# google-research/se3ds

Hardware: AMD Instinct MI355X
Metric: panoramas/sec (G+D train step) at 512x1024 RGB-D (higher is better)
Workload: dtype bf16; 1 GPU; configs/highres 512x1024 full GAN step train_g_d (G+D+hinge+depth+wc losses, clip, Adam, EMA), ResNet-101 gen_dims 128, per-GPU batch 8, d_step_per_g_step 1; per_gpu_batch=8, global_batch=8, parallelism=dp1

## Files before the change

### include/se3ds_hip.h

```cpp
#ifndef SE3DS_HIP_H_
#define SE3DS_HIP_H_

#include <stddef.h>
#include <stdint.h>

#ifdef __cplusplus
extern "C" {
#endif

#define SE3DS_OK 0
#define SE3DS_E_BADSHAPE (-1)
#define SE3DS_E_BADDTYPE (-2)
#define SE3DS_E_WORKSPACE (-3)
#define SE3DS_E_LAUNCH (-4)
#define SE3DS_E_UNSUPPORTED (-5)

#define SE3DS_F32 0
#define SE3DS_I32 1
#define SE3DS_U8 2
#define SE3DS_BF16 3
#define SE3DS_FEAT_BYTE_RANGE 0x100
#define SE3DS_XYZ1_ONES_PRESET 0x200

const char* se3ds_version(void);
// ... 237 lines not shown
                         void* stream);
int se3ds_upsample2x_fwd(const void* x, int dtype, int n, int h, int w, int c, void* y,
                         void* stream);
int se3ds_upsample2x_bwd(const void* dy, int dtype, int n, int h, int w, int c, void* dx,
                         void* stream);
int se3ds_copy_channels(const void* src, int src_dtype, int src_c, int src_c0, void* dst,
                        int dst_dtype, int dst_c, int dst_c0, int ncopy, int64_t rows,
                        void* stream);
int se3ds_fill(void* p, int dtype, int64_t n, float value, void* stream);
int se3ds_quantize(const void* in, int in_dtype, int64_t n, int pre_clamp, float pre_lo,
                   float pre_hi, float mul, float div, float lo, float hi, void* out, int out_dtype,
                   void* stream);
int se3ds_pad2d(const void* x, int dtype, int n, int h, int w, int c, int pad, int mode, int wrap_w,
                float value, void* y, void* stream);
int se3ds_head_fwd(const void* x, int dtype, int64_t n, int kind, float* y, void* stream);
int se3ds_head_bwd(const float* dy, const float* y, const void* x, int dtype, int64_t n, int kind,
                   void* dx, void* stream);

int se3ds_sample_sum(const float* a, const float* b, const float* m, int n, int64_t p, int c,
                     int mode, float* out, float* workspace , void* stream);
int se3ds_l1_grad(const float* a, const float* b, const float* m, const float* m2,
                  const float* coef, int n, int64_t p, int c, int mode, float* grad, void* stream);
int se3ds_recip_clamp(const float* sums, int n, float scale, float* out, void* stream);
int se3ds_hinge(const void* logits, int dtype, int64_t half, float cd, float cg, float* sums,
                void* dlog_d, void* dlog_g, void* stream);

int se3ds_multi_sqnorm(const float* grads, const int64_t* chunks, int64_t nchunks,
                       const int64_t* tensor_chunk_start, int ntensors, float* partial,
                       float* sqnorm, void* stream);
int se3ds_multi_clip_by_norm(float* grads, const int64_t* chunks, int64_t nchunks,
                             const float* sqnorm, int ntensors, float clip_norm,
                             float* mean_norm_out, void* stream);
int se3ds_mean_clipped_norm(const float* sqnorm, int ntensors, float clip_norm, float* out,
                            void* stream);
int se3ds_multi_adam_keras(float* params, const float* grads, float* m, float* v, int64_t n,
                           float lr, float beta1, float beta2, float eps, int64_t step,
                           void* stream);
int se3ds_multi_adam_keras_ema(float* params, const float* grads, float* m, float* v, int64_t n,
                               float lr, float beta1, float beta2, float eps, int64_t step,
                               float* ema, float one_minus_decay, void* stream);
int se3ds_multi_clip_adam_keras_ema(float* params, const float* grads, float* m, float* v,
                                    const int64_t* chunks, int64_t nchunks, const float* sqnorm,
                                    float clip_norm, const int64_t* tensor_sn, float lr, float beta1,
                                    float beta2, float eps, int64_t step, float* ema,
                                    float one_minus_decay, void* stream);
int se3ds_multi_ema(float* ema, const float* vars, int64_t n, float one_minus_decay, void* stream);

int se3ds_spectral_table_fields(void);
int se3ds_spectral_part_rows(void);
int se3ds_spectral_vpart_len(void);
int se3ds_spectral_power_iter(const int64_t* table, int nlayers, int training, void* stream);
int se3ds_spectral_bwd_fixup(const int64_t* table, int nlayers, void* stream);
int se3ds_spectral_bwd_dots(const int64_t* table, int nlayers, void* stream);
int se3ds_multi_sqnorm_sn(const float* grads, const int64_t* chunks, int64_t nchunks,
                          const int64_t* tensor_chunk_start, int ntensors, float* partial,
                          float* sqnorm, const int64_t* tensor_sn, int tensor_base, void* stream);
int se3ds_multi_clip_by_norm_sn(float* grads, const int64_t* chunks, int64_t nchunks,
                                const float* sqnorm, int ntensors, float clip_norm,
                                float* mean_norm_out, const int64_t* tensor_sn, void* stream);


int se3ds_input_transform(const uint8_t* image, const uint8_t* proj_image, const uint16_t* depth,
                          const uint16_t* proj_depth, const uint8_t* proj_mask,
                          const uint8_t* blurred_mask, const uint8_t* segmentation,
                          const int32_t* iparams, const float* fparams, int n, int h0, int w0, int h,
                          int w, float* o_image, float* o_proj_image, float* o_proj_mask,
                          float* o_proj_depth, float* o_depth, float* o_blurred, int32_t* o_seg,
                          void* stream);

int se3ds_video_transform(const float* image, const uint8_t* segmentation,
                          const uint8_t* pd_segmentation, const float* depth, const float* pd_depth,
                          const int32_t* hmode, const float* hband, int n, int t, int h0, int w0,
                          int h, int w, float* o_original, float* o_image, uint8_t* o_seg,
                          uint8_t* o_pd_seg, float* o_depth, float* o_pd_depth, void* stream);

int se3ds_re10k_extent(const uint8_t* visible_mask, int n, int h0, int w0, int32_t* extents,
                       void* stream);
int se3ds_re10k_extent_vector_bytes(const uint8_t* visible_mask, int w0);

int se3ds_re10k_transform(const uint8_t* image, const uint8_t* proj_image, const uint16_t* depth,
                          const uint16_t* proj_depth, const uint8_t* proj_mask,
                          const uint8_t* visible_mask, const uint8_t* segmentation,
                          const int32_t* extents, const int32_t* iparams, const float* fparams,
                          int n, int h0, int w0, int h, int w, float* o_image, float* o_proj_image,
                          float* o_proj_mask, float* o_proj_depth, float* o_depth, float* o_blurred,
                          int32_t* o_seg, int32_t* o_bbox, int32_t* o_status, void* stream);

int se3ds_png_unfilter(const uint8_t* src, int64_t src_bytes, const int64_t* table,
                       const int64_t* host_table, int n, void* stream);
int se3ds_png_unfilter_fields(void);
int se3ds_png_unfilter_max_row_bytes(void);

int se3ds_png_inflate(const uint8_t* buf, int64_t buf_bytes, uint8_t* workspace,
                      int64_t workspace_bytes, const int64_t* host_table, int n,
                      int32_t* status_dev, void* stream);
int se3ds_png_inflate_fields(void);
int se3ds_png_inflate_ring_bytes(void);

int se3ds_jpeg_decode(const uint8_t* buf, int64_t buf_bytes, uint8_t* workspace,
                      int64_t workspace_bytes, const int64_t* host_images, int n_images,
                      const int64_t* host_segments, int n_segments, int32_t* status_dev, int phases,
                      void* stream);
size_t se3ds_jpeg_decode_workspace_bytes(const int64_t* host_images, int n_images);
int se3ds_jpeg_decode_fields(void);
int se3ds_jpeg_decode_segment_fields(void);
int se3ds_jpeg_decode_lanes(void);
// ... 167 lines not shown
```

### se3ds_amd/csrc/optim.hip

```cpp
#include "common.h"
#include <cmath>

namespace se3ds {
namespace {

constexpr int kB = 256;

__global__ void __launch_bounds__(kB)
chunk_sqsum_kernel(const float* __restrict__ g, const int64_t* __restrict__ chunks,
                   float* __restrict__ partial, const int64_t* __restrict__ tensor_sn) {
  __shared__ float sh[kB / 64];
  const int64_t start = chunks[blockIdx.x * 3 + 1], len = chunks[blockIdx.x * 3 + 2];
  if (tensor_sn && tensor_sn[chunks[blockIdx.x * 3]] != 0) {
    if (threadIdx.x == 0) partial[blockIdx.x] = 0.f;
    return;
  }
  float s = 0.f;
  const float* gp = g + start;
  const int64_t n4 = (((uintptr_t)gp & 15) == 0) ? (len >> 2) : 0;
  float s1 = 0.f, s2 = 0.f, s3 = 0.f;
  for (int64_t i = threadIdx.x; i < n4; i += kB) {
    const float4 v = reinterpret_cast<const float4*>(gp)[i];
    s += v.x * v.x;
    s1 += v.y * v.y;
// ... 310 lines not shown
  }
  dot = wave_sum(dot);
  __syncthreads();
  if ((threadIdx.x & 63) == 0) sh[threadIdx.x >> 6] = dot;
  __syncthreads();
  if (threadIdx.x == 0) {
    float sigma = (sh[0] + sh[1]) + (sh[2] + sh[3]);
    sig[0] = sigma;
    sig[1] = 1.0f / (sigma + SN_EPS);
  }
  float vn = 0.f;
  for (int i = 0; i < SN_RB; ++i) vn += vpart[i];
  const float inv_vn = 1.0f / (sqrtf(vn) + SN_EPS);
  for (int64_t k = threadIdx.x; k < K; k += kB) v[k] = v[k] * inv_vn;
}

__global__ void __launch_bounds__(kB)
sn_dot_kernel(const int64_t* __restrict__ tab) {
  const int64_t* L = tab + (int64_t)blockIdx.y * SN_F;
  const float* W = (const float*)L[0];
  float* vpart = (float*)L[6];
  const float* G = (const float*)L[9];
  const int64_t n = L[7] * L[8];
  __shared__ float sh[kB / 64];
  float s = 0.f;
  for (int64_t i = (int64_t)blockIdx.x * kB + threadIdx.x; i < n; i += (int64_t)SN_RB * kB)
    s += G[i] * W[i];
  s = wave_sum(s);
  if ((threadIdx.x & 63) == 0) sh[threadIdx.x >> 6] = s;
  __syncthreads();
  if (threadIdx.x == 0) vpart[blockIdx.x] = (sh[0] + sh[1]) + (sh[2] + sh[3]);
}

__global__ void __launch_bounds__(kB)
sn_fix_kernel(const int64_t* __restrict__ tab) {
  const int64_t* L = tab + (int64_t)blockIdx.y * SN_F;
  const float* v = (const float*)L[2];
  const float* uhat = (const float*)L[3];
  const float* sig = (const float*)L[4];
  const float* vpart = (const float*)L[6];
  float* G = (float*)L[9];
  const int C = (int)L[8];
  const int64_t n = L[7] * C;
  const float dot = sn_dot_gw(vpart);
  const float inv = sig[1];
  const float coef = inv * inv * dot;
  for (int64_t i = (int64_t)blockIdx.x * kB + threadIdx.x; i < n; i += (int64_t)SN_RB * kB) {
    int64_t k = i / C;
    int c = (int)(i - k * C);
    G[i] = inv * G[i] - coef * v[k] * uhat[c];
  }
}

__global__ void __launch_bounds__(kB)
sn_dots_kernel(const int64_t* __restrict__ tab) {
  const int64_t* L = tab + (int64_t)blockIdx.y * SN_F;
  const float* W = (const float*)L[0];
  const float* v = (const float*)L[2];
  const float* uhat = (const float*)L[3];
  float* vpart = (float*)L[6];
  const float* G = (const float*)L[9];
  const int64_t K = L[7];
  const int C = (int)L[8];
  __shared__ float sh[3][kB / 64];
  const int lane = threadIdx.x & 63, wave = threadIdx.x >> 6;
  float dot = 0.f, gg = 0.f, gvu = 0.f;
  const bool vec = (C & 3) == 0 && ((((uintptr_t)G | (uintptr_t)W | (uintptr_t)uhat) & 15) == 0);
  for (int64_t k = (int64_t)blockIdx.x * 4 + wave; k < K; k += (int64_t)SN_RB * 4) {
    const float vk = v[k];
    float row = 0.f;
    if (vec) {
      const float4* G4 = reinterpret_cast<const float4*>(G + k * C);
      const float4* W4 = reinterpret_cast<const float4*>(W + k * C);
      const float4* U4 = reinterpret_cast<const float4*>(uhat);
      for (int c = lane; c < (C >> 2); c += 64) {
        const float4 gv = G4[c], wv = W4[c], uv = U4[c];
        dot += (gv.x * wv.x + gv.y * wv.y) + (gv.z * wv.z + gv.w * wv.w);
        gg += (gv.x * gv.x + gv.y * gv.y) + (gv.z * gv.z + gv.w * gv.w);
        row += (gv.x * uv.x + gv.y * uv.y) + (gv.z * uv.z + gv.w * uv.w);
      }
    } else {
      for (int c = lane; c < C; c += 64) {
        const float gv = G[k * C + c];
        dot += gv * W[k * C + c];
        gg += gv * gv;
        row += gv * uhat[c];
      }
    }
    gvu += row * vk;
  }
  dot = wave_sum(dot);
  gg = wave_sum(gg);
  gvu = wave_sum(gvu);
  if (lane == 0) { sh[0][wave] = dot; sh[1][wave] = gg; sh[2][wave] = gvu; }
  __syncthreads();
  if (threadIdx.x < 3) {
    const float* q = sh[threadIdx.x];
    vpart[threadIdx.x * SN_RB + blockIdx.x] = (q[0] + q[1]) + (q[2] + q[3]);
  }
  if (blockIdx.x == 0) {
    __syncthreads();
    float nv = 0.f, nu = 0.f;
    for (int64_t k = threadIdx.x; k < K; k += kB) nv += v[k] * v[k];
    for (int c = threadIdx.x; c < C; c += kB) nu += uhat[c] * uhat[c];
    nv = wave_sum(nv);
    nu = wave_sum(nu);
    if (lane == 0) { sh[0][wave] = nv; sh[1][wave] = nu; }
    __syncthreads();
    if (threadIdx.x < 2) {
      const float* q = sh[threadIdx.x];
      vpart[3 * SN_RB + threadIdx.x] = (q[0] + q[1]) + (q[2] + q[3]);
    }
  }
}

__global__ void __launch_bounds__(kB)
sn_sqnorm_kernel(const int64_t* __restrict__ tensor_sn, int tensor_base, int T,
                 float* __restrict__ sqnorm) {
  for (int t = blockIdx.x * kB + threadIdx.x; t < T; t += gridDim.x * kB) {
    const int64_t* L = (const int64_t*)tensor_sn[tensor_base + t];
    if (L == nullptr) continue;
    const float* sig = (const float*)L[4];
    const float* vpart = (const float*)L[6];
    const float dot = sn_dot_gw(vpart);
    double gg = 0.0, gvu = 0.0;
    for (int i = 0; i < SN_RB; ++i) {
      gg += (double)vpart[SN_RB + i];
      gvu += (double)vpart[2 * SN_RB + i];
    }
// ... 88 lines not shown
  float alpha = adam_alpha(lr, beta1, beta2, step);
  hipLaunchKernelGGL(adam_ema_kernel, dim3(grid_for(n, kB)), dim3(kB), 0, as_stream(stream), params,
                     grads, m, v, n, alpha, beta1, beta2, eps, ema, one_minus_decay);
  return check_launch("multi_adam_keras_ema");
}

int se3ds_multi_clip_adam_keras_ema(float* params, const float* grads, float* m, float* v,
                                    const int64_t* chunks, int64_t nchunks, const float* sqnorm,
                                    float clip_norm, const int64_t* tensor_sn, float lr, float beta1,
                                    float beta2, float eps, int64_t step, float* ema,
                                    float one_minus_decay, void* stream) {
  if (nchunks <= 0) return SE3DS_OK;
  if ((((uintptr_t)params | (uintptr_t)grads | (uintptr_t)m | (uintptr_t)v | (uintptr_t)ema) & 15) != 0)
    return SE3DS_E_UNSUPPORTED;
  const float alpha = adam_alpha(lr, beta1, beta2, step);
  if (ema)
    hipLaunchKernelGGL(clip_adam_kernel<true>, dim3((unsigned)nchunks), dim3(kB), 0, as_stream(stream),
                       params, grads, m, v, chunks, sqnorm, clip_norm, tensor_sn, alpha, beta1, beta2,
                       eps, ema, one_minus_decay);
  else
    hipLaunchKernelGGL(clip_adam_kernel<false>, dim3((unsigned)nchunks), dim3(kB), 0, as_stream(stream),
                       params, grads, m, v, chunks, sqnorm, clip_norm, tensor_sn, alpha, beta1, beta2,
                       eps, ema, one_minus_decay);
  return check_launch("multi_clip_adam_keras_ema");
}

int se3ds_multi_ema(float* ema, const float* vars, int64_t n, float one_minus_decay,
                    void* stream) {
  if (n <= 0) return SE3DS_OK;
  hipLaunchKernelGGL(ema_kernel, dim3(grid_for(n, kB)), dim3(kB), 0, as_stream(stream), ema, vars,
                     n, one_minus_decay);
  return check_launch("multi_ema");
}

int se3ds_spectral_power_iter(const int64_t* table, int nlayers, int training, void* stream) {
  if (nlayers <= 0) return SE3DS_OK;
  hipStream_t s = as_stream(stream);
  hipLaunchKernelGGL(sn_v_kernel, dim3(SN_RB, (unsigned)nlayers), dim3(kB), 0, s, table);
  hipLaunchKernelGGL(sn_u_kernel, dim3(SN_KB, (unsigned)nlayers), dim3(kB), 0, s, table);
  hipLaunchKernelGGL(sn_finish_kernel, dim3((unsigned)nlayers), dim3(kB), 0, s, table, training);
  return check_launch("spectral_power_iter");
}

int se3ds_spectral_bwd_fixup(const int64_t* table, int nlayers, void* stream) {
  if (nlayers <= 0) return SE3DS_OK;
  hipStream_t s = as_stream(stream);
  hipLaunchKernelGGL(sn_dot_kernel, dim3(SN_RB, (unsigned)nlayers), dim3(kB), 0, s, table);
  hipLaunchKernelGGL(sn_fix_kernel, dim3(SN_RB, (unsigned)nlayers), dim3(kB), 0, s, table);
  return check_launch("spectral_bwd_fixup");
}

int se3ds_spectral_bwd_dots(const int64_t* table, int nlayers, void* stream) {
  if (nlayers <= 0) return SE3DS_OK;
  hipLaunchKernelGGL(sn_dots_kernel, dim3(SN_RB, (unsigned)nlayers), dim3(kB), 0, as_stream(stream),
                     table);
  return check_launch("spectral_bwd_dots");
}

int se3ds_spectral_table_fields(void) { return SN_F; }
int se3ds_spectral_part_rows(void) { return SN_KB; }
int se3ds_spectral_vpart_len(void) { return 3 * SN_RB + 2; }

}
```

### se3ds_amd/hipops/nn.py

```python
import math
import threading
from collections import namedtuple
from types import SimpleNamespace
from typing import List, Optional

import numpy as np
import os

import torch
import torch.distributed as dist

from se3ds_amd import _lib

ACT_NONE, ACT_RELU, ACT_LRELU = 0, 1, 2
BN_EPS, BN_MOMENTUM = 1e-3, 0.99
IN_EPS = 1e-3


def _L():
  return _lib.lib()


def _all_reduce_sum(t, group, kind):
  from se3ds_amd.trainers import dist_utils
# ... 164 lines not shown
    self.grad_scaled = None
    self.requires_grad = requires_grad
    self.col_stats = None
    self.grad_pre_act = False
    self.shared = False
    self.grad_ev = None

  @property
  def shape(self):
    return self.data.shape

  @property
  def grad(self):
    return self._grad

  @grad.setter
  def grad(self, g):
    self._grad = g
    self.gver += 1

  def take_bn_stats(self):
    s, self.bn_stats = self.bn_stats, None
    return s.rows if s is not None and s.gver == self.gver else None

  def take_grad_scaled(self, who):
    gs = self.grad_scaled
    if gs is not None and gs != self.gver:
      raise RuntimeError(f'{who}: pre-scaled output gradient was modified by a second '
                         'consumer (set SE3DS_FUSED_ROW_SCALE=0)')
    self.grad_scaled = None
    return gs is not None


class Ctx:

  def __init__(self, device, dtype=torch.float32, training=False, record=False,
               group=None, world=None):
    self.device = torch.device(device)
    self.dtype = dtype
    self.code = _lib.dtype_code(torch.empty(0, dtype=dtype))
    self.training = training
    self.tape = [] if record else None
    self.param_grads = True
    self.binary_masks = True
    self.on_segment = None
    self.batch_limit = None
    self.act_taps = None
    self.taps = None
    self.bn_use_moving = False
    self.after_collective = None
    self._mask_cache = {}
    self.streams = None
    self.wgrad_defer = None
    self._tl = threading.local()
    self._forked = set()
    self.pair = None
    self.collectives = 0
    self._bwd_pending = None
    self._cur_paired = False
    self.group = group
    if world is None:
      world = dist.get_world_size(group) if group is not None else 1
    self.world = int(world)
    if group is not None and self.world != dist.get_world_size(group):
      raise ValueError(f'Ctx: world={self.world} does not match the replica group '
                       f'({dist.get_world_size(group)} ranks)')
    if group is None and self.world > 1 and not (dist.is_initialized() and
                                                 dist.get_world_size() == self.world):
      raise ValueError(f'Ctx: world={self.world} without a group needs a default process group '
                       'of that size')
    self._ws = {}

  def ws(self, key, nbytes):
    if self.streams is not None:
      key = (key, torch.cuda.current_stream(self.device).cuda_stream)
    elif self.pair is not None:
      key = (key, self.branch_tag)
    t = self._ws.get(key)
    if t is None or t.numel() < nbytes:
      t = torch.empty((int(nbytes),), dtype=torch.uint8, device=self.device)
      self._ws[key] = t
    return t

  def empty(self, shape, dtype=None):
    return torch.empty(shape, dtype=dtype or self.dtype, device=self.device)

  @property
  def branch_tag(self):
    return getattr(self._tl, 'tag', 0)

  @branch_tag.setter
  def branch_tag(self, tag):
    self._tl.tag = tag

  def record(self, fn, sync=False):
    if self.tape is not None:
      self.tape.append((fn, self.branch_tag, 1 if sync else 0))

  def run_branches(self, fns):
    if self.world > 1 and len(fns) == 2:
      return _run_paired(self, fns)
    out = {}
    for tag, fn in fns.items():
      with self.branch(tag):
        out[tag] = fn()
    self.join()
    return out

  def branch(self, tag):
    return _Branch(self, tag)

  def join(self):
    if self._forked and self.streams is not None:
      main = torch.cuda.current_stream(self.device)
      for tag in sorted(self._forked):
        main.wait_stream(self.streams[tag])
      self._forked.clear()

  def backward(self):
    tape, self.tape = self.tape, []
    if self.world > 1:
      tape = _merge_paired(tape)
    self._replay(tape)

  def _replay(self, tape):
    cur, scope = 0, None
    try:
      for fn, tag, sync in reversed(tape):
        self._cur_paired = sync == 2
        t = tag if self.streams is not None else 0
        if t != cur:
          flush_wgrad_reduces(self)
          if scope is not None:
            scope.__exit__(None, None, None)
            scope = None
          if t == 0:
            self.join()
          else:
            scope = self.branch(t)
            scope.__enter__()
          cur = t
        fn()
      flush_wgrad_reduces(self)
    finally:
      if scope is not None:
        scope.__exit__(None, None, None)
      self._cur_paired = False
      pending, self._bwd_pending = self._bwd_pending, None
      self.join()
    assert pending is None, 'unpaired SyncBN backward'

  def mark_segment(self, name):
    if self.tape is not None:
      def fire():
        if self.on_segment is not None and self.param_grads:
          self.on_segment(name)
      self.tape.append((fire, self.branch_tag, 0))

  def _allreduce_joint(self, a, b):
    buf = torch.cat([a.reshape(-1), b.reshape(-1)])
    _all_reduce_sum(buf, self.group, 'syncbn_pair')
    a.copy_(buf[:a.numel()].view_as(a))
    b.copy_(buf[a.numel():].view_as(b))
    self._after_collective()

  def _after_collective(self):
    self.collectives += 1
    if self.after_collective is not None:
      self.after_collective()

  def allreduce_sum(self, t):
    if self.world > 1:
      pair = self.pair
      if pair is not None and self.branch_tag:
        pair.allreduce(t, self.branch_tag)
        return
      _all_reduce_sum(t, self.group, 'syncbn')
      self._after_collective()

  def allreduce_then(self, t, cont):
    if self.world > 1:
      if self._cur_paired:
        on_streams = self.streams is not None and t.is_cuda
        if self._bwd_pending is None:
          ev = None
          if on_streams:
            ev = torch.cuda.Event()
            ev.record()
          self._bwd_pending = (t, cont, ev, self.branch_tag)
          return
        t0, cont0, ev0, tag0 = self._bwd_pending
        self._bwd_pending = None
        if ev0 is not None:
          torch.cuda.current_stream(self.device).wait_event(ev0)
        self._allreduce_joint(t0, t)
        if ev0 is not None and tag0 != self.branch_tag:
# ... 340 lines not shown
      K, co = w.shape[0] * w.shape[1] * w.shape[2], w.shape[3]
      if dtype == torch.bfloat16 and K % 8 == 0 and co % 4 == 0:
        ent = l._copies.get(dtype)
        if ent is None:
          wt = torch.empty((co, K), dtype=dtype, device=w.device)
          wn = torch.empty((K, co), dtype=dtype, device=w.device)
          l._copies[dtype] = (-1, wt, wn)
        else:
          wt, wn = ent[1], ent[2]
        if (w.data_ptr() | wt.data_ptr()) % 16 == 0 and wn.data_ptr() % 8 == 0:
          rows.append([w.data_ptr(), K, co, wt.data_ptr(), wn.data_ptr(), tile0])
          tile0 += ((K + 63) // 64) * ((co + 63) // 64)
          self.batched.append(l)
          continue
      self.single.append(l)
    self.tiles = tile0
    self.table = torch.tensor(rows, dtype=torch.int64, device=device) if rows else None

  def prep(self, version):
    if self.table is not None:
      _chk(_L().se3ds_weight_prep_multi(self.table.data_ptr(), len(self.batched), self.tiles,
                                        _lib.stream()), 'se3ds_weight_prep_multi')
      for l in self.batched:
        ent = l._copies[self.dtype]
        l._copies[self.dtype] = (version, ent[1], ent[2])
    for l in self.single:
      l.prep(self.dtype, version)


class SpectralGroup:

  def __init__(self, layers: List[ConvLayer], device):
    self.layers = [l for l in layers if l.spectral]
    L = _L()
    nf, pr, vl = (L.se3ds_spectral_table_fields(), L.se3ds_spectral_part_rows(),
                  L.se3ds_spectral_vpart_len())
    rows = []
    for l in self.layers:
      w = l.kernel
      K, co = w.shape[0] * w.shape[1] * w.shape[2], w.shape[3]
      l.sn = dict(v=torch.zeros(K, device=device), uhat=torch.zeros(co, device=device),
                  sig=torch.ones(2, device=device), part=torch.zeros(pr * co, device=device),
                  vpart=torch.zeros(vl, device=device))
      rows.append([w.data_ptr(), l.store[l.name + '/u'].data_ptr(), l.sn['v'].data_ptr(),
                   l.sn['uhat'].data_ptr(), l.sn['sig'].data_ptr(), l.sn['part'].data_ptr(),
                   l.sn['vpart'].data_ptr(), K, co, 0])
      assert len(rows[-1]) == nf
    self._rows = rows
    self.table = torch.tensor(rows, dtype=torch.int64, device=device) if rows else None
    self._eff = [i for i, l in enumerate(self.layers) if l.kind == 'spectral']
    self._eff_table = None
    self._tensor_sn = None
    self._seg_tables = {}

  @property
  def eff_table(self):
    if self._eff_table is None and self._eff:
      rows = []
      for i in self._eff:
        l = self.layers[i]
        r = list(self._rows[i])
        r[9] = l.store.grad_views[l.name + '/kernel'].data_ptr()
        rows.append(r)
      self._eff_table = torch.tensor(rows, dtype=torch.int64, device=self.table.device)
    return self._eff_table

  def power_iteration(self, training):
    if self.table is not None:
      _chk(_L().se3ds_spectral_power_iter(self.table.data_ptr(), self.table.shape[0],
                                          1 if training else 0, _lib.stream()),
           'se3ds_spectral_power_iter')

  def tensor_sn(self, store):
    tab = self.eff_table
    if tab is None:
      return None
    if self._tensor_sn is None:
      nf = tab.shape[1]
      index = {n_: t for t, n_ in enumerate(store.trainable_names)}
      rows = [0] * len(store.trainable_names)
      for j, i in enumerate(self._eff):
        rows[index[self.layers[i].name + '/kernel']] = tab.data_ptr() + 8 * nf * j
      self._tensor_sn = torch.tensor(rows, dtype=torch.int64, device=tab.device)
    return self._tensor_sn

  def backward_fixup(self, prefix=None, dots_only=False):
    tab = self.eff_table
    if tab is None:
      return
    if prefix is not None:
      cache = self._seg_tables
      if prefix not in cache:
        pres = prefix if isinstance(prefix, (tuple, list)) else (prefix,)
        rows = [j for j, i in enumerate(self._eff)
                if any(self.layers[i].name.startswith(pre + '/') for pre in pres)]
        cache[prefix] = tab[rows].contiguous() if rows else None
      tab = cache[prefix]
      if tab is None:
        return
    if dots_only:
      _chk(_L().se3ds_spectral_bwd_dots(tab.data_ptr(), tab.shape[0], _lib.stream()),
           'se3ds_spectral_bwd_dots')
      return
    _chk(_L().se3ds_spectral_bwd_fixup(tab.data_ptr(), tab.shape[0], _lib.stream()),
         'se3ds_spectral_bwd_fixup')


_CHECK_MASKS = os.environ.get('SE3DS_CHECK_MASKS') == '1'


def mask_window(ctx, mask, n, h, w, ho, wo, k, stride, pad_t, pad_l, wrap, want_bwd):
  if _CHECK_MASKS and ctx.binary_masks and not bool(((mask == 0) | (mask == 1)).all()):
    raise _lib.Se3dsHipError('a partial-conv mask with values outside {0, 1} reached a binary-mask fast path: '
                             'set gan.binary_masks = False (ctx.binary_masks) for fractional masks')
  ratio = torch.empty((n, ho, wo), dtype=torch.float32, device=ctx.device)
  um = torch.empty_like(ratio)
  ru = torch.empty_like(ratio) if want_bwd else None
  bu = torch.empty_like(ratio) if want_bwd else None
  _chk(_L().se3ds_mask_window(mask.data_ptr(), n, h, w, ho, wo, k, k, stride, pad_t, pad_l,
                              1 if wrap else 0, ratio.data_ptr(), um.data_ptr(), _lib.ptr(ru),
                              _lib.ptr(bu), _lib.stream()), 'se3ds_mask_window')
  return ratio, um, ru, bu


def _colsum(ctx, t2d_ptr, dtype_code, rows, c, row_scale=None, groups=1, out=None):
  sums = torch.empty((groups, 2, c), dtype=torch.float32, device=ctx.device)
  L = _L()
  ws = ctx.ws('norm', L.se3ds_norm_workspace_bytes(groups, c))
  _chk(L.se3ds_norm_stats(t2d_ptr, dtype_code, groups, rows, c, _lib.ptr(row_scale),
                          sums.data_ptr(), _lib.ptr(out), ws.data_ptr(), ws.numel(),
                          _lib.stream()), 'se3ds_norm_stats')
  return sums


_RED_TABLES = {}


def _wgrad(ctx, layer, args, wsz):
  L = _L()
  if ctx.wgrad_defer is None:
    ws = _global_ws(ctx.device, 'wgrad', wsz)
    _chk(L.se3ds_conv2d_wgrad(*args, None, 0, ws.data_ptr(), ws.numel(), _lib.stream()),
         'se3ds_conv2d_wgrad')
    return
  ws = layer._wgrad_slab
  if ws is None or ws.numel() < wsz:
    ws = torch.empty((int(wsz),), dtype=torch.uint8, device=ctx.device)
    layer._wgrad_slab = ws
    _RED_TABLES.clear()
  row = (_lib.c_i64 * 5)()
  _chk(L.se3ds_conv2d_wgrad_partial(*args, ws.data_ptr(), ws.numel(), row, _lib.stream()),
       'se3ds_conv2d_wgrad_partial')
  if row[4]:
    ctx.wgrad_defer.append((row[0], row[1], row[2], row[3]))


def flush_wgrad_reduces(ctx):
  rows = ctx.wgrad_defer
  if not rows:
    return
  ctx.wgrad_defer = []
  _reduce_rows(ctx, rows)


def reduce_or_defer(ctx, row):
  if ctx.wgrad_defer is not None:
    ctx.wgrad_defer.append(row)
  else:
    _reduce_rows(ctx, [row])


def _reduce_rows(ctx, rows):
  key = (str(ctx.device), tuple(rows))
  ent = _RED_TABLES.get(key)
  if ent is None:
    tile = int(_L().se3ds_wgrad_reduce_tile())
    tab, first = [], 0
    for part, splits, n4, dst in rows:
      tab.append([part, splits, n4, dst, first])
      first += (n4 + tile - 1) // tile
    ent = (torch.tensor(tab, dtype=torch.int64, device=ctx.device), first)
    if len(_RED_TABLES) >= 256:
      _RED_TABLES.clear()
    _RED_TABLES[key] = ent
  with _Timed('wgrad', 0.0, 'split reduce (batched)'):
    _chk(_L().se3ds_wgrad_reduce_multi(ent[0].data_ptr(), len(rows), ent[1], _lib.stream()),
         'se3ds_wgrad_reduce_multi')


_Geom = namedtuple('_Geom', 'code n h w cin ho wo cout kh kw stride pad_t pad_l wrap')

def _partial_masks(ctx, mask, geo, recording):
  _, n, h, w, _, ho, wo, _, k, _, s, pt, pl, wrap = geo
  m = in_mask = mask
  if m is None:
    m = torch.empty((n, h, w), dtype=torch.float32, device=ctx.device)
    _chk(_L().se3ds_fill(m.data_ptr(), _lib.F32, m.numel(), 1.0, _lib.stream()), 'se3ds_fill')
  cache = ctx._mask_cache if mask is not None else None
  key = (m.data_ptr(), tuple(m.shape), k, s, pt, pl, wrap, ho, wo, bool(recording))
  ent = cache.get(key) if cache is not None and _MASK_CACHE else None
  if ent is None:
    ratio, um, ru, bu = mask_window(ctx, m, n, h, w, ho, wo, k, s, pt, pl, wrap, recording)
    if (cache is not None and _MASK_CACHE and ctx.binary_masks and k == 1 and s == 1 and pt == 0 and
        pl == 0):
      um = m
    if cache is not None:
      cache[key] = (ratio, um, ru, bu, m)
  else:
    ratio, um, ru, bu = ent[:4]
  if in_mask is not None and k == 1 and ctx.binary_masks and _DROP_1X1_MASK:
    in_mask = None
  return ratio, um, ru, bu, in_mask


# ... 561 lines not shown
```

### se3ds_amd/trainers/se3ds_trainer.py

```python
import os
from typing import Dict

import torch

from se3ds_amd import _lib
from se3ds_amd import gin_lite as gin
from se3ds_amd.hipops import nn
from se3ds_amd.hipops.nn import Var
from se3ds_amd.models import image_models
from se3ds_amd.trainers import dist_utils
from se3ds_amd.trainers import gan_manager
from se3ds_amd.trainers.gan_manager import Mean

FUSED_SN_CLIP = True
GRAD_CLIP_NORM = 5.0
SEGMENT_OPTIMIZER = os.environ.get('SE3DS_SEGMENT_OPTIMIZER', '1') != '0'
FUSED_CLIP_ADAM = os.environ.get('SE3DS_FUSED_CLIP_ADAM', '1') != '0'
DEFER_WGRAD_REDUCE = os.environ.get('SE3DS_DEFER_WGRAD_REDUCE', '1') != '0'


def _L():
  return _lib.lib()


@gin.configurable(denylist=['strategy', 'model_dir'])
class GAN(gan_manager.GANManager):

  def __init__(self, lambda_gan, lambda_kld, lambda_wc, lambda_depth, *args,
               dis_use_pred_depth=True, mask_blurred=False, **kwargs):
    super().__init__(*args, **kwargs)
    self.lambda_gan = lambda_gan
    self.lambda_kld = lambda_kld
    self.lambda_wc = lambda_wc
    self.lambda_depth = lambda_depth
    self.dis_use_pred_depth = dis_use_pred_depth
    self.mask_blurred = mask_blurred

  def _create_metrics(self):
    names = ['gen/gen_loss', 'dis/disc_loss', 'dis/grad_norm', 'gen/gen_feat_loss',
             'gen/gen_gan_loss', 'gen/depth_loss', 'gen/seg_loss', 'gen/depth_seg_loss',
             'gen/depth_seg_consistency', 'gen/kld_loss', 'gen/kld_nan', 'gen/wc_loss',
             'gen/grad_norm']
    self.metrics = {n: Mean(n.split('/')[-1]) for n in names}

  def _prep_inputs(self, inputs):
    inputs = dict(inputs)
    for k in ('image', 'proj_image', 'proj_depth', 'proj_mask', 'depth', 'blurred_mask'):
      t = inputs[k]
      _lib.require_cuda(t)
      inputs[k] = t.to(torch.float32).contiguous()
    if not self.mask_blurred:
      bm = torch.empty_like(inputs['blurred_mask'])
      _lib.check(_L().se3ds_fill(bm.data_ptr(), _lib.F32, bm.numel(), 0.0, _lib.stream()),
                 'se3ds_fill')
      inputs['blurred_mask'] = bm
    return inputs

  def _disc_input(self, ctx, generated, depth_out, image, depth):
    n = image.shape[0]
    fake_d = depth_out if self.dis_use_pred_depth else depth
    fake = nn.concat_channels(ctx, [generated, fake_d])
    real = nn.concat_channels(ctx, [image, depth])
    x = ctx.empty((2 * n,) + tuple(fake.shape[1:]))
    x[:n].copy_(fake)
    x[n:].copy_(real)
    return Var(x, requires_grad=False)

  def _run_discriminator(self, ctx, x_all):
    res = self.discriminator.forward(ctx, x_all)
    return res

# ... 156 lines not shown
    self._set_input_grad(x_all, False)
    self._backward_tape(ctx_d, tape_d, seeds_d, logits)
    D.spectral.backward_fixup()
    if sync is not None:
      d_norm = self._sync_discriminator(sync)
    ctx_d.param_grads = False
    ctx_d.batch_limit = n
    self._set_input_grad(x_all, True)
    self._backward_tape(ctx_d, tape_d, [g[:n] for g in seeds_g], logits)
    ctx_d.batch_limit = None
    gx = x_all.grad
    x_all.grad = None
    del tape_d
    g_rgb = nn.slice_channels(gx[:n], 0, 3, torch.float32)
    _lib.check(L.se3ds_add(d_rgb.data_ptr(), g_rgb.data_ptr(), _lib.F32, d_rgb.numel(),
                           d_rgb.data_ptr(), _lib.stream()), 'se3ds_add')
    if self.dis_use_pred_depth:
      g_dep = nn.slice_channels(gx[:n], 3, 1, torch.float32)
      _lib.check(L.se3ds_add(d_depth.data_ptr(), g_dep.data_ptr(), _lib.F32, d_depth.numel(),
                             d_depth.data_ptr(), _lib.stream()), 'se3ds_add')
    ctx_g.param_grads = True
    push_rgb(d_rgb)
    push_depth(d_depth)
    ema_theta, ema_omd = self.ema_fused_args()
    if sync is None and SEGMENT_OPTIMIZER and nn.conv_profiler() is None:
      segs = self._segments()
      opt = self._optimizer_stream(dev)
      main = torch.cuda.current_stream(dev)
      ev = torch.cuda.Event()
      ev.record()
      with torch.cuda.stream(opt):
        opt.wait_event(ev)
        self._update_all(self.d_optimizer, False, None, 0.0)
        d_norm = self.d_optimizer.mean_clipped_norm(GRAD_CLIP_NORM).clone()
      self.g_optimizer.begin_step()
      def segment_done(name):
        if name not in segs:
          return
        t0, t1, e0, e1 = segs[name]
        done = torch.cuda.Event()
        done.record()
        with torch.cuda.stream(opt):
          opt.wait_event(done)
          nn.flush_wgrad_reduces(ctx_g)
          G.spectral.backward_fixup(prefix=G.SEGMENTS[name], dots_only=FUSED_SN_CLIP)
          if not (FUSED_CLIP_ADAM and self.g_optimizer.clip_apply(
              t0, t1, GRAD_CLIP_NORM, FUSED_SN_CLIP, ema_theta, ema_omd)):
            self.g_optimizer.clip_segment(t0, t1, GRAD_CLIP_NORM, fused_sn=FUSED_SN_CLIP)
            self.g_optimizer.apply_segment(e0, e1, ema_theta, ema_omd)
          self._operand_group(G, name, ctx_g.dtype).prep(G.store.version + 1)
      ctx_g.on_segment = segment_done
      if DEFER_WGRAD_REDUCE:
        ctx_g.wgrad_defer = []
      ctx_g.backward()
      ctx_g.on_segment = None
      ctx_g.wgrad_defer = None
      with torch.cuda.stream(opt):
        opt.wait_stream(main)
        self._operand_group(D, None, ctx_d.dtype).prep(D.store.version)
      main.wait_stream(opt)
      self.g_optimizer.end_step()
      g_norm = self.g_optimizer.mean_clipped_norm(GRAD_CLIP_NORM).clone()
    elif sync is None:
      if DEFER_WGRAD_REDUCE:
        ctx_g.wgrad_defer = []
      ctx_g.backward()
      ctx_g.wgrad_defer = None
      G.spectral.backward_fixup(dots_only=FUSED_SN_CLIP)
      self._update_all(self.g_optimizer, FUSED_SN_CLIP, ema_theta, ema_omd)
      g_norm = self.g_optimizer.mean_clipped_norm(GRAD_CLIP_NORM).clone()
      self._update_all(self.d_optimizer, False, None, 0.0)
      d_norm = self.d_optimizer.mean_clipped_norm(GRAD_CLIP_NORM).clone()
      self._operand_group(G, None, ctx_g.dtype).prep(G.store.version)
      self._operand_group(D, None, ctx_d.dtype).prep(D.store.version)
    else:
      opt = self._optimizer_stream(dev)
      main = torch.cuda.current_stream(dev)
      opt.wait_stream(main)
      def segment_done(name):
        if name not in self._g_segments:
          return
        t0, t1, e0, e1 = self._g_segments[name]
        done = torch.cuda.Event()
        done.record()
        with torch.cuda.stream(opt):
          opt.wait_event(done)
          nn.flush_wgrad_reduces(ctx_g)
          G.spectral.backward_fixup(prefix=G.SEGMENTS[name], dots_only=FUSED_SN_CLIP)
          self.g_optimizer.clip_segment(t0, t1, GRAD_CLIP_NORM, fused_sn=FUSED_SN_CLIP)
          sync.reduce_range(G.store.grad, e0, e1)
      ctx_g.on_segment = segment_done
      ctx_g.after_collective = sync.pump
      if DEFER_WGRAD_REDUCE:
        ctx_g.wgrad_defer = []
      ctx_g.backward()
      ctx_g.on_segment = None
      ctx_g.after_collective = None
      ctx_g.wgrad_defer = None
      main.wait_stream(opt)
      g_norm = self.g_optimizer.mean_clipped_norm(GRAD_CLIP_NORM).clone()
      sync.finish()
      self.g_optimizer.apply_gradients(group, 1, ema_theta, ema_omd)
      self.d_optimizer.apply_gradients(group, 1)
    self.last_collectives = ctx_g.collectives
    if self.global_step == 0:
      self.ema_generator.forward(self.ema_generator.make_ctx(training=True, group=group, world=R), inputs)
    self.update_ema_model(theta_done=ema_theta is not None)

    lam_d = self.lambda_depth if self.predict_depth else 0.0
    def gen_gan():
      return self.lambda_gan * sum(float(s[0]) / c for s, c in hinge_sums) / n_dis
    def disc():
      return self.lambda_gan * sum(float(s[1]) / c for s, c in hinge_sums) / n_dis
    def depth_loss():
      return lam_d * float((depth_l1 / torch.clamp(npx, min=1)).mean())
    def wc_loss():
      return self.lambda_wc * float((wc_l1 / 3.0 / torch.clamp(wcm, min=1)).mean())
    self.metrics['dis/disc_loss'].update_state(disc)
    self.metrics['dis/grad_norm'].update_state(d_norm)
    self.metrics['gen/gen_gan_loss'].update_state(gen_gan)
    self.metrics['gen/gen_loss'].update_state(lambda: gen_gan() + depth_loss() + wc_loss())
    self.metrics['gen/depth_loss'].update_state(depth_loss)
    self.metrics['gen/seg_loss'].update_state(0.0)
    self.metrics['gen/depth_seg_loss'].update_state(0.0)
    self.metrics['gen/depth_seg_consistency'].update_state(0.0)
    self.metrics['gen/kld_loss'].update_state(0.0)
    self.metrics['gen/kld_nan'].update_state(0.0)
    self.metrics['gen/wc_loss'].update_state(wc_loss)
    self.metrics['gen/grad_norm'].update_state(g_norm)

  def _update_all(self, opt, fused_sn, ema_theta, ema_omd):
    nt = len(opt.model.store.trainable_names)
    opt.begin_step()
    if not (FUSED_CLIP_ADAM and opt.clip_apply(0, nt, GRAD_CLIP_NORM, fused_sn, ema_theta, ema_omd)):
      opt.iterations -= 1
      opt.clip_gradients(GRAD_CLIP_NORM, fused_sn=fused_sn)
      opt.apply_gradients(None, 1, ema_theta, ema_omd)
    else:
      opt.end_step()

  def _set_input_grad(self, x_all, flag):
    x_all.requires_grad = flag
    for v in getattr(self.discriminator, '_scale_inputs', []):
      v.requires_grad = flag

  def train_d(self, inputs: Dict[str, torch.Tensor]) -> None:
    inputs = self._prep_inputs(inputs)
    image, depth_t = inputs['image'], inputs['depth']
    R = self.strategy.num_replicas_in_sync
# ... 25 lines not shown
```

Measured before the change: 41.99 panoramas/sec.

## Fuse split-K weight-gradient slab reduction into spectral-norm backward dots kernel

For spectral-normalized conv layers, the deferred split-K weight-gradient partial reduction is parked instead of run as a separate reduce. The spectral-norm dots kernel then sums the partial slabs, writes the reduced gradient, and computes its dot products in the same pass. This removes one full read/write pass over those gradients and some launches. In exchange it adds parking bookkeeping across backward, segment flushes and trainer paths, and relies on alignment checks and fixed summation order to keep results unchanged.

```diff
diff --git a/include/se3ds_hip.h b/include/se3ds_hip.h
--- a/include/se3ds_hip.h
+++ b/include/se3ds_hip.h
@@ -313,6 +313,8 @@
 int se3ds_spectral_power_iter(const int64_t* table, int nlayers, int training, void* stream);
 int se3ds_spectral_bwd_fixup(const int64_t* table, int nlayers, void* stream);
 int se3ds_spectral_bwd_dots(const int64_t* table, int nlayers, void* stream);
+int se3ds_spectral_bwd_dots_slabs(const int64_t* table, int nlayers, const int64_t* slab_rows,
+                                  void* stream);
 int se3ds_multi_sqnorm_sn(const float* grads, const int64_t* chunks, int64_t nchunks,
                           const int64_t* tensor_chunk_start, int ntensors, float* partial,
                           float* sqnorm, const int64_t* tensor_sn, int tensor_base, void* stream);
diff --git a/se3ds_amd/csrc/optim.hip b/se3ds_amd/csrc/optim.hip
--- a/se3ds_amd/csrc/optim.hip
+++ b/se3ds_amd/csrc/optim.hip
@@ -386,8 +386,36 @@
   }
 }
 
-__global__ void __launch_bounds__(kB)
-sn_dots_kernel(const int64_t* __restrict__ tab) {
+__device__ __forceinline__ float slab_fold(float s0, float s1, float s2, float s3) {
+  return __fmul_rn(__fadd_rn(__fadd_rn(s0, s1), __fadd_rn(s2, s3)), 1.0f);
+}
+__device__ __forceinline__ float4 slab_sum4(const float4* __restrict__ P, int splits, int64_t n4,
+                                            int64_t i) {
+  float4 s0 = make_float4(0.f, 0.f, 0.f, 0.f), s1 = s0, s2 = s0, s3 = s0;
+  auto add = [](float4& a, const float4& b) {
+    a.x = __fadd_rn(a.x, b.x); a.y = __fadd_rn(a.y, b.y);
+    a.z = __fadd_rn(a.z, b.z); a.w = __fadd_rn(a.w, b.w);
+  };
+  if (splits == 2) {
+    const float4 a = P[i], b = P[n4 + i];
+    add(s0, a);
+    add(s0, b);
+  } else {
+    int k = 0;
+    for (; k + 3 < splits; k += 4) {
+      const float4 a = P[(int64_t)k * n4 + i], b = P[(int64_t)(k + 1) * n4 + i];
+      const float4 c = P[(int64_t)(k + 2) * n4 + i], d = P[(int64_t)(k + 3) * n4 + i];
+      add(s0, a); add(s1, b); add(s2, c); add(s3, d);
+    }
+    for (; k < splits; ++k) add(s0, P[(int64_t)k * n4 + i]);
+  }
+  return make_float4(slab_fold(s0.x, s1.x, s2.x, s3.x), slab_fold(s0.y, s1.y, s2.y, s3.y),
+                     slab_fold(s0.z, s1.z, s2.z, s3.z), slab_fold(s0.w, s1.w, s2.w, s3.w));
+}
+
+template <bool SLABS>
+__global__ void __launch_bounds__(kB)
+sn_dots_kernel(const int64_t* __restrict__ tab, const int64_t* __restrict__ slab_rows) {
   const int64_t* L = tab + (int64_t)blockIdx.y * SN_F;
   const float* W = (const float*)L[0];
   const float* v = (const float*)L[2];
@@ -400,6 +428,14 @@
   const int lane = threadIdx.x & 63, wave = threadIdx.x >> 6;
   float dot = 0.f, gg = 0.f, gvu = 0.f;
   const bool vec = (C & 3) == 0 && ((((uintptr_t)G | (uintptr_t)W | (uintptr_t)uhat) & 15) == 0);
+  const float4* P = nullptr;
+  int splits = 0;
+  if (SLABS) {
+    P = reinterpret_cast<const float4*>(slab_rows[(int64_t)blockIdx.y * 2]);
+    splits = (int)slab_rows[(int64_t)blockIdx.y * 2 + 1];
+    if (!vec || (((uintptr_t)P) & 15) != 0) P = nullptr;
+  }
+  const int64_t n4 = (K * C) >> 2;
   for (int64_t k = (int64_t)blockIdx.x * 4 + wave; k < K; k += (int64_t)SN_RB * 4) {
     const float vk = v[k];
     float row = 0.f;
@@ -408,7 +444,14 @@
       const float4* W4 = reinterpret_cast<const float4*>(W + k * C);
       const float4* U4 = reinterpret_cast<const float4*>(uhat);
       for (int c = lane; c < (C >> 2); c += 64) {
-        const float4 gv = G4[c], wv = W4[c], uv = U4[c];
+        float4 gv;
+        if (SLABS && P != nullptr) {
+          gv = slab_sum4(P, splits, n4, k * (C >> 2) + c);
+          reinterpret_cast<float4*>(const_cast<float*>(G) + k * C)[c] = gv;
+        } else {
+          gv = G4[c];
+        }
+        const float4 wv = W4[c], uv = U4[c];
         dot += (gv.x * wv.x + gv.y * wv.y) + (gv.z * wv.z + gv.w * wv.w);
         gg += (gv.x * gv.x + gv.y * gv.y) + (gv.z * gv.z + gv.w * gv.w);
         row += (gv.x * uv.x + gv.y * uv.y) + (gv.z * uv.z + gv.w * uv.w);
@@ -603,9 +646,18 @@
 
 int se3ds_spectral_bwd_dots(const int64_t* table, int nlayers, void* stream) {
   if (nlayers <= 0) return SE3DS_OK;
-  hipLaunchKernelGGL(sn_dots_kernel, dim3(SN_RB, (unsigned)nlayers), dim3(kB), 0, as_stream(stream),
-                     table);
+  hipLaunchKernelGGL(sn_dots_kernel<false>, dim3(SN_RB, (unsigned)nlayers), dim3(kB), 0,
+                     as_stream(stream), table, (const int64_t*)nullptr);
   return check_launch("spectral_bwd_dots");
+}
+
+int se3ds_spectral_bwd_dots_slabs(const int64_t* table, int nlayers, const int64_t* slab_rows,
+                                  void* stream) {
+  if (nlayers <= 0) return SE3DS_OK;
+  if (slab_rows == nullptr) return se3ds_spectral_bwd_dots(table, nlayers, stream);
+  hipLaunchKernelGGL(sn_dots_kernel<true>, dim3(SN_RB, (unsigned)nlayers), dim3(kB), 0,
+                     as_stream(stream), table, slab_rows);
+  return check_launch("spectral_bwd_dots_slabs");
 }
 
 int se3ds_spectral_table_fields(void) { return SN_F; }
diff --git a/se3ds_amd/hipops/nn.py b/se3ds_amd/hipops/nn.py
--- a/se3ds_amd/hipops/nn.py
+++ b/se3ds_amd/hipops/nn.py
@@ -240,6 +240,8 @@
     self._mask_cache = {}
     self.streams = None
     self.wgrad_defer = None
+    self.sn_dots_slabs = False
+    self._sn_parked = []
     self._tl = threading.local()
     self._forked = set()
     self.pair = None
@@ -305,20 +307,20 @@
         main.wait_stream(self.streams[tag])
       self._forked.clear()
 
-  def backward(self):
+  def backward(self, keep_parked=False):
     tape, self.tape = self.tape, []
     if self.world > 1:
       tape = _merge_paired(tape)
-    self._replay(tape)
-
-  def _replay(self, tape):
+    self._replay(tape, keep_parked)
+
+  def _replay(self, tape, keep_parked=False):
     cur, scope = 0, None
     try:
       for fn, tag, sync in reversed(tape):
         self._cur_paired = sync == 2
         t = tag if self.streams is not None else 0
         if t != cur:
-          flush_wgrad_reduces(self)
+          flush_wgrad_reduces(self, parked=True)
           if scope is not None:
             scope.__exit__(None, None, None)
             scope = None
@@ -329,7 +331,7 @@
             scope.__enter__()
           cur = t
         fn()
-      flush_wgrad_reduces(self)
+      flush_wgrad_reduces(self, parked=not keep_parked)
     finally:
       if scope is not None:
         scope.__exit__(None, None, None)
@@ -776,6 +778,7 @@
     self._eff_table = None
     self._tensor_sn = None
     self._seg_tables = {}
+    self._slab_tabs = {}
 
   @property
   def eff_table(self):
@@ -812,15 +815,23 @@
     tab = self.eff_table
     if tab is None:
       return
+    layers = [self.layers[i] for i in self._eff]
     if prefix is not None:
       cache = self._seg_tables
       if prefix not in cache:
         pres = prefix if isinstance(prefix, (tuple, list)) else (prefix,)
         rows = [j for j, i in enumerate(self._eff)
                 if any(self.layers[i].name.startswith(pre + '/') for pre in pres)]
-        cache[prefix] = tab[rows].contiguous() if rows else None
-      tab = cache[prefix]
-      if tab is None:
+        cache[prefix] = (tab[rows].contiguous(), [layers[j] for j in rows]) if rows else None
+      if cache[prefix] is None:
+        return
+      tab, layers = cache[prefix]
+    slabs = self._slab_rows(prefix, layers)
+    if slabs is not None:
+      with _Timed('wgrad', 0.0, 'split reduce (in the spectral dots)'):
+        _chk(_L().se3ds_spectral_bwd_dots_slabs(tab.data_ptr(), tab.shape[0], slabs.data_ptr(),
+                                                _lib.stream()), 'se3ds_spectral_bwd_dots_slabs')
+      if dots_only:
         return
     if dots_only:
       _chk(_L().se3ds_spectral_bwd_dots(tab.data_ptr(), tab.shape[0], _lib.stream()),
@@ -828,6 +839,16 @@
       return
     _chk(_L().se3ds_spectral_bwd_fixup(tab.data_ptr(), tab.shape[0], _lib.stream()),
          'se3ds_spectral_bwd_fixup')
+
+  def _slab_rows(self, key, layers):
+    rows = tuple((l.sn.pop('slab_row', None) or (0, 0))[:2] for l in layers)
+    if not any(p for p, _ in rows):
+      return None
+    ent = self._slab_tabs.get(key)
+    if ent is None or ent[0] != rows:
+      ent = (rows, torch.tensor(rows, dtype=torch.int64, device=self.table.device))
+      self._slab_tabs[key] = ent
+    return ent[1]
 
 
 _CHECK_MASKS = os.environ.get('SE3DS_CHECK_MASKS') == '1'
@@ -867,6 +888,8 @@
     _chk(L.se3ds_conv2d_wgrad(*args, None, 0, ws.data_ptr(), ws.numel(), _lib.stream()),
          'se3ds_conv2d_wgrad')
     return
+  if layer.sn is not None and layer.sn.get('slab_row') is not None:
+    _reduce_rows(ctx, [layer.sn.pop('slab_row')])
   ws = layer._wgrad_slab
   if ws is None or ws.numel() < wsz:
     ws = torch.empty((int(wsz),), dtype=torch.uint8, device=ctx.device)
@@ -876,14 +899,37 @@
   _chk(L.se3ds_conv2d_wgrad_partial(*args, ws.data_ptr(), ws.numel(), row, _lib.stream()),
        'se3ds_conv2d_wgrad_partial')
   if row[4]:
-    ctx.wgrad_defer.append((row[0], row[1], row[2], row[3]))
-
-
-def flush_wgrad_reduces(ctx):
-  rows = ctx.wgrad_defer
+    r = (row[0], row[1], row[2], row[3])
+    if ctx.sn_dots_slabs and _dots_take_slabs(layer, r):
+      layer.sn['slab_row'] = r
+      ctx._sn_parked.append(layer)
+    else:
+      ctx.wgrad_defer.append(r)
+
+
+def _dots_take_slabs(layer, row):
+  if layer.kind != 'spectral' or layer.sn is None:
+    return False
+  w = layer.kernel
+  g = layer.store.grad_views[layer.name + '/kernel']
+  return (row[3] == g.data_ptr() and 4 * row[2] == w.numel() and w.shape[3] % 4 == 0 and
+          (row[0] | row[3] | w.data_ptr() | layer.sn['uhat'].data_ptr()) % 16 == 0)
+
+
+def _take_parked(ctx):
+  rows = [l.sn.pop('slab_row') for l in ctx._sn_parked if l.sn.get('slab_row') is not None]
+  ctx._sn_parked = []
+  return rows
+
+
+def flush_wgrad_reduces(ctx, parked=False):
+  rows = ctx.wgrad_defer or []
+  if parked and ctx._sn_parked:
+    rows = list(rows) + _take_parked(ctx)
   if not rows:
     return
-  ctx.wgrad_defer = []
+  if ctx.wgrad_defer is not None:
+    ctx.wgrad_defer = []
   _reduce_rows(ctx, rows)
 
 
diff --git a/se3ds_amd/trainers/se3ds_trainer.py b/se3ds_amd/trainers/se3ds_trainer.py
--- a/se3ds_amd/trainers/se3ds_trainer.py
+++ b/se3ds_amd/trainers/se3ds_trainer.py
@@ -17,6 +17,7 @@
 SEGMENT_OPTIMIZER = os.environ.get('SE3DS_SEGMENT_OPTIMIZER', '1') != '0'
 FUSED_CLIP_ADAM = os.environ.get('SE3DS_FUSED_CLIP_ADAM', '1') != '0'
 DEFER_WGRAD_REDUCE = os.environ.get('SE3DS_DEFER_WGRAD_REDUCE', '1') != '0'
+SN_DOTS_SLABS = True
 
 
 def _L():
@@ -279,8 +280,10 @@
       ctx_g.on_segment = segment_done
       if DEFER_WGRAD_REDUCE:
         ctx_g.wgrad_defer = []
+        ctx_g.sn_dots_slabs = SN_DOTS_SLABS
       ctx_g.backward()
       ctx_g.on_segment = None
+      ctx_g.sn_dots_slabs = False
       ctx_g.wgrad_defer = None
       with torch.cuda.stream(opt):
         opt.wait_stream(main)
@@ -291,9 +294,12 @@
     elif sync is None:
       if DEFER_WGRAD_REDUCE:
         ctx_g.wgrad_defer = []
-      ctx_g.backward()
+        ctx_g.sn_dots_slabs = SN_DOTS_SLABS
+      ctx_g.backward(keep_parked=True)
       ctx_g.wgrad_defer = None
+      ctx_g.sn_dots_slabs = False
       G.spectral.backward_fixup(dots_only=FUSED_SN_CLIP)
+      nn.flush_wgrad_reduces(ctx_g, parked=True)
       self._update_all(self.g_optimizer, FUSED_SN_CLIP, ema_theta, ema_omd)
       g_norm = self.g_optimizer.mean_clipped_norm(GRAD_CLIP_NORM).clone()
       self._update_all(self.d_optimizer, False, None, 0.0)
@@ -320,8 +326,10 @@
       ctx_g.after_collective = sync.pump
       if DEFER_WGRAD_REDUCE:
         ctx_g.wgrad_defer = []
+        ctx_g.sn_dots_slabs = SN_DOTS_SLABS
       ctx_g.backward()
       ctx_g.on_segment = None
+      ctx_g.sn_dots_slabs = False
       ctx_g.after_collective = None
       ctx_g.wgrad_defer = None
       main.wait_stream(opt)
```

Measured after the change: 42.13 panoramas/sec, median of 6. Within noise of the previous version (+0.3%).
